# dronefreak/CABiNet

Hardware: AMD Instinct MI355X
Metric: 1024x1024 images/sec fwd+bwd (CABiNet-MobileNetV3-Large) (higher is better)
Workload: dtype f32; 1 GPU; BASELINE configs[2]: CABiNet-MobileNetV3-Large, 8x3x1024x1024 synthetic 8-class per GPU, fwd + 2x OhemCE + bwd + grad all-reduce + SGD step, HIP CAB/FFM kernels, fp32, random-init (model seed 0, gamma=0.5); per_gpu_batch=8, global_batch=8, n_classes=8, parallelism=dp1, miopen_find_mode=FAST

## Files before the change

### cabinet_amd/csrc/pwconv.hip

```cpp
#include "common.hpp"

namespace cabinet {

constexpr int PW_MAXB = 4;

template <int MB>
__global__ __launch_bounds__(64) void pw_stream_kernel(const float* __restrict__ a, int sm, int sk, int M, int K,
                                                        const float* __restrict__ x, int P, int nblocks,
                                                        int blocks_per_img, float* __restrict__ y) {
    extern __shared__ __attribute__((aligned(16))) float al[];
    const int lane = threadIdx.x, li = lane & 31, h = lane >> 5, ld = K + 1;
    for (int i0 = 0; i0 < 32 * MB * K; i0 += 64 * 8) {
        float v[8];
#pragma unroll
        for (int j = 0; j < 8; ++j) {
            const int i = i0 + j * 64 + lane, m = i / K, k = i - m * K;
            v[j] = (i < 32 * MB * K && m < M) ? a[(size_t)m * sm + (size_t)k * sk] : 0.f;
        }
#pragma unroll
        for (int j = 0; j < 8; ++j) {
            const int i = i0 + j * 64 + lane, m = i / K, k = i - m * K;
            if (i < 32 * MB * K) al[m * ld + k] = v[j];
        }
    }
    __syncthreads();
    for (int blk = blockIdx.x; blk < nblocks; blk += gridDim.x) {
        const int b = blk / blocks_per_img, p0 = (blk - b * blocks_per_img) * 64;
        const float* xb = x + (size_t)b * K * P;
        const int pa = min(p0 + li, P - 1), pb = min(p0 + 32 + li, P - 1);
        f32x16 acc[MB][2];
#pragma unroll
        for (int i = 0; i < MB; ++i)
#pragma unroll
            for (int j = 0; j < 2; ++j)
#pragma unroll
                for (int r = 0; r < 16; ++r) acc[i][j][r] = 0.f;
        for (int k0 = 0; k0 < K; k0 += 8) {
            float b0[4], b1[4];
#pragma unroll
            for (int s = 0; s < 4; ++s) {
                const float* row = xb + (size_t)(k0 + 2 * s + h) * P;
                b0[s] = row[pa];
                b1[s] = row[pb];
            }
#pragma unroll
            for (int s = 0; s < 4; ++s) {
#pragma unroll
                for (int i = 0; i < MB; ++i) {
                    const float av = al[(32 * i + li) * ld + k0 + 2 * s + h];
                    acc[i][0] = mfma32(av, b0[s], acc[i][0]);
                    acc[i][1] = mfma32(av, b1[s], acc[i][1]);
                }
            }
        }
        float* yb = y + (size_t)b * M * P;
#pragma unroll
        for (int i = 0; i < MB; ++i)
#pragma unroll
            for (int r = 0; r < 16; ++r) {
                const int m = 32 * i + acc_row(r) + 4 * h;
                if (m < M) {
                    if (p0 + li < P) yb[(size_t)m * P + p0 + li] = acc[i][0][r];
                    if (p0 + 32 + li < P) yb[(size_t)m * P + p0 + 32 + li] = acc[i][1][r];
                }
            }
    }
}

template <int COB, int CIB>
__global__ __launch_bounds__(64) void pw_wgrad_kernel(const float* __restrict__ dy, const float* __restrict__ x, int Co,
                                                       int Ci, int P, int nchunks, int chunks_per_img,
                                                       float* __restrict__ slabs) {
    extern __shared__ __attribute__((aligned(16))) float tl[];
    float* ty = tl;
    float* tx = tl + 32 * COB * 65;
    const int lane = threadIdx.x, li = lane & 31, h = lane >> 5;
    for (int i = lane; i < (32 * COB + 32 * CIB) * 65; i += 64) tl[i] = 0.f;
    f32x16 acc[COB][CIB];
#pragma unroll
    for (int i = 0; i < COB; ++i)
#pragma unroll
        for (int j = 0; j < CIB; ++j)
#pragma unroll
            for (int r = 0; r < 16; ++r) acc[i][j][r] = 0.f;
    for (int ch = blockIdx.x; ch < nchunks; ch += gridDim.x) {
        const int b = ch / chunks_per_img, p0 = (ch - b * chunks_per_img) * 64;
        const bool live = p0 + lane < P;
        const float* dyb = dy + (size_t)b * Co * P + p0 + lane;
        const float* xb = x + (size_t)b * Ci * P + p0 + lane;
        __syncthreads();
        auto stage = [&](const float* src, float* dst, int rows) {
            for (int r0 = 0; r0 < rows; r0 += 16) {
                float v[16];
#pragma unroll
                for (int j = 0; j < 16; ++j) v[j] = (live && r0 + j < rows) ? src[(size_t)(r0 + j) * P] : 0.f;
#pragma unroll
                for (int j = 0; j < 16; ++j)
                    if (r0 + j < rows) dst[(r0 + j) * 65 + lane] = v[j];
            }
        };
        stage(dyb, ty, Co);
        stage(xb, tx, Ci);
        __syncthreads();
#pragma unroll 4
        for (int s = 0; s < 32; ++s) {
            float av[COB], bv[CIB];
#pragma unroll
            for (int i = 0; i < COB; ++i) av[i] = ty[(32 * i + li) * 65 + 2 * s + h];
#pragma unroll
            for (int j = 0; j < CIB; ++j) bv[j] = tx[(32 * j + li) * 65 + 2 * s + h];
#pragma unroll
            for (int i = 0; i < COB; ++i)
#pragma unroll
                for (int j = 0; j < CIB; ++j) acc[i][j] = mfma32(av[i], bv[j], acc[i][j]);
        }
    }
    float* slab = slabs + (size_t)blockIdx.x * Co * Ci;
#pragma unroll
    for (int i = 0; i < COB; ++i)
#pragma unroll
        for (int j = 0; j < CIB; ++j)
#pragma unroll
            for (int r = 0; r < 16; ++r) {
                const int co = 32 * i + acc_row(r) + 4 * h, ci = 32 * j + li;
                if (co < Co && ci < Ci) slab[(size_t)co * Ci + ci] = acc[i][j][r];
            }
}

__global__ __launch_bounds__(256) void pw_slab_sum_kernel(const float* __restrict__ slabs, int nslab, int count,
                                                           float* __restrict__ dw) {
    const int i = blockIdx.x * 4 + (threadIdx.x >> 6), lane = threadIdx.x & 63;
    if (i >= count) return;
    float s0 = 0.f, s1 = 0.f;
    int k = lane;
    for (; k + 64 < nslab; k += 128) {
        s0 += slabs[(size_t)k * count + i];
        s1 += slabs[(size_t)(k + 64) * count + i];
    }
    if (k < nslab) s0 += slabs[(size_t)k * count + i];
    const float t = wave_sum(s0 + s1);
    if (lane == 0) dw[i] = t;
}

static int blocks_of(int n) { return ceil_div(n, 32); }
constexpr int PW_GRID = 256 * 8;

bool pwconv_supported(int Ci, int Co, int P) {
    (void)P;
    return Ci % 8 == 0 && Co % 8 == 0 && Ci <= 32 * PW_MAXB && Co <= 32 * PW_MAXB &&
           blocks_of(Ci) * blocks_of(Co) <= 8 && 32 * PW_MAXB * (Ci > Co ? Ci + 1 : Co + 1) * 4 <= 64 * 1024;
}

static int wgrad_slabs(int B, int P) {
    const int nchunks = B * ceil_div(P, 64);
    return nchunks < PW_GRID ? nchunks : PW_GRID;
}
size_t pwconv_bwd_workspace(int B, int Ci, int Co, int P) {
    return align_up((size_t)wgrad_slabs(B, P) * Co * Ci * sizeof(float), 256);
}

static hipError_t stream_launch(const float* a, int sm, int sk, int M, int K, const float* x, int B, int P, float* y,
                                hipStream_t stream) {
    const int bpi = ceil_div(P, 64), nblocks = B * bpi, grid = nblocks < PW_GRID ? nblocks : PW_GRID;
    const int mb = blocks_of(M);
    const size_t lds = (size_t)32 * mb * (K + 1) * sizeof(float);
#define PW_STREAM(MBV)                                                                                               \
    hipLaunchKernelGGL(pw_stream_kernel<MBV>, dim3(grid), dim3(64), lds, stream, a, sm, sk, M, K, x, P, nblocks, bpi, y)
    if (mb == 1) PW_STREAM(1);
    else if (mb == 2) PW_STREAM(2);
    else if (mb == 3) PW_STREAM(3);
    else PW_STREAM(4);
#undef PW_STREAM
    return hipGetLastError();
}

hipError_t pwconv_fwd_run(const float* x, const float* w, int B, int Ci, int Co, int P, float* y, hipStream_t stream) {
    return stream_launch(w, Ci, 1, Co, Ci, x, B, P, y, stream);
}

template <int COB>
static void wgrad_launch_ci(int cib, int grid, size_t lds, hipStream_t stream, const float* dy, const float* x, int Co,
                            int Ci, int P, int nchunks, int cpi, float* slabs) {
#define PW_WG(CIBV)                                                                                                    \
    hipLaunchKernelGGL((pw_wgrad_kernel<COB, CIBV>), dim3(grid), dim3(64), lds, stream, dy, x, Co, Ci, P, nchunks, cpi, \
                       slabs)
    if (cib == 1) PW_WG(1);
    else if (cib == 2) PW_WG(2);
    else if (cib == 3) { if constexpr (COB <= 2) PW_WG(3); }
    else { if constexpr (COB <= 2) PW_WG(4); }
#undef PW_WG
}

hipError_t pwconv_bwd_run(const float* dy, const float* x, const float* w, int B, int Ci, int Co, int P, float* dx,
                          float* dw, void* ws, hipStream_t stream) {
    if (dx) {
        hipError_t e = stream_launch(w, 1, Ci, Ci, Co, dy, B, P, dx, stream);
        if (e != hipSuccess) return e;
    }
    if (dw) {
        const int cpi = ceil_div(P, 64), nchunks = B * cpi, grid = wgrad_slabs(B, P);
        const int cob = blocks_of(Co), cib = blocks_of(Ci);
        const size_t lds = (size_t)(32 * cob + 32 * cib) * 65 * sizeof(float);
        float* slabs = static_cast<float*>(ws);
        if (cob == 1) wgrad_launch_ci<1>(cib, grid, lds, stream, dy, x, Co, Ci, P, nchunks, cpi, slabs);
        else if (cob == 2) wgrad_launch_ci<2>(cib, grid, lds, stream, dy, x, Co, Ci, P, nchunks, cpi, slabs);
        else if (cob == 3) wgrad_launch_ci<3>(cib, grid, lds, stream, dy, x, Co, Ci, P, nchunks, cpi, slabs);
        else wgrad_launch_ci<4>(cib, grid, lds, stream, dy, x, Co, Ci, P, nchunks, cpi, slabs);
        hipLaunchKernelGGL(pw_slab_sum_kernel, dim3(ceil_div(Co * Ci, 4)), dim3(256), 0, stream, slabs, grid, Co * Ci, dw);
    }
    return hipGetLastError();
}

}
```

Baseline: 364.1 images/s.

## Software-pipeline pointwise conv streaming loads and add opt-in fused backward kernel

```diff
diff --git a/cabinet_amd/csrc/pwconv.hip b/cabinet_amd/csrc/pwconv.hip
--- a/cabinet_amd/csrc/pwconv.hip
+++ b/cabinet_amd/csrc/pwconv.hip
@@ -1,4 +1,5 @@
 #include "common.hpp"
+#include "slab_sum.hpp"
 
 namespace cabinet {
 
@@ -24,47 +25,230 @@
         }
     }
     __syncthreads();
-    for (int blk = blockIdx.x; blk < nblocks; blk += gridDim.x) {
+    int lblk = blockIdx.x, lk = 0, lpa = 0, lpb = 0;
+    const float* lxb = x;
+    const int row_bytes = P * (int)sizeof(float);
+    auto set_block = [&](int blk) {
         const int b = blk / blocks_per_img, p0 = (blk - b * blocks_per_img) * 64;
-        const float* xb = x + (size_t)b * K * P;
-        const int pa = min(p0 + li, P - 1), pb = min(p0 + 32 + li, P - 1);
-        f32x16 acc[MB][2];
+        lpa = (h * P + min(p0 + li, P - 1)) * 4, lpb = (h * P + min(p0 + 32 + li, P - 1)) * 4;
+        lxb = x + (size_t)b * K * P;
+    };
+    set_block(lblk);
+    auto load = [&](float (&b0)[4], float (&b1)[4]) {
+        const buf_rsrc r = make_rsrc(lxb + (size_t)lk * P, 0xffffffffu);
+#pragma unroll
+        for (int s = 0; s < 4; ++s) {
+            b0[s] = bload(r, lpa, 2 * s * row_bytes);
+            b1[s] = bload(r, lpb, 2 * s * row_bytes);
+        }
+        lk += 8;
+        if (lk == K) {
+            lk = 0;
+            if (lblk + (int)gridDim.x < nblocks) set_block(lblk += gridDim.x);
+        }
+    };
+    int cblk = blockIdx.x, ck = 0;
+    f32x16 acc[MB][2];
+    auto compute = [&](const float (&b0)[4], const float (&b1)[4]) {
+        if (cblk >= nblocks) return;
+        if (ck == 0) {
+#pragma unroll
+            for (int i = 0; i < MB; ++i)
+#pragma unroll
+                for (int j = 0; j < 2; ++j)
+#pragma unroll
+                    for (int r = 0; r < 16; ++r) acc[i][j][r] = 0.f;
+        }
+#pragma unroll
+        for (int s = 0; s < 4; ++s) {
+#pragma unroll
+            for (int i = 0; i < MB; ++i) {
+                const float av = al[(32 * i + li) * ld + ck + 2 * s + h];
+                acc[i][0] = mfma32(av, b0[s], acc[i][0]);
+                acc[i][1] = mfma32(av, b1[s], acc[i][1]);
+            }
+        }
+        ck += 8;
+        if (ck < K) return;
+        const int b = cblk / blocks_per_img, p0 = (cblk - b * blocks_per_img) * 64;
+        float* yb = y + (size_t)b * M * P;
+        const unsigned so = 4u * h * P + p0 + li;
 #pragma unroll
         for (int i = 0; i < MB; ++i)
 #pragma unroll
-            for (int j = 0; j < 2; ++j)
-#pragma unroll
-                for (int r = 0; r < 16; ++r) acc[i][j][r] = 0.f;
-        for (int k0 = 0; k0 < K; k0 += 8) {
-            float b0[4], b1[4];
-#pragma unroll
-            for (int s = 0; s < 4; ++s) {
-                const float* row = xb + (size_t)(k0 + 2 * s + h) * P;
-                b0[s] = row[pa];
-                b1[s] = row[pb];
-            }
-#pragma unroll
-            for (int s = 0; s < 4; ++s) {
-#pragma unroll
-                for (int i = 0; i < MB; ++i) {
-                    const float av = al[(32 * i + li) * ld + k0 + 2 * s + h];
-                    acc[i][0] = mfma32(av, b0[s], acc[i][0]);
-                    acc[i][1] = mfma32(av, b1[s], acc[i][1]);
+            for (int r = 0; r < 16; ++r) {
+                if (32 * i + 8 * (r >> 2) < M) {
+                    float* row = yb + (size_t)(32 * i + acc_row(r)) * P;
+                    if (p0 + li < P) row[so] = acc[i][0][r];
+                    if (p0 + 32 + li < P) row[so + 32] = acc[i][1][r];
                 }
             }
-        }
-        float* yb = y + (size_t)b * M * P;
-#pragma unroll
-        for (int i = 0; i < MB; ++i)
+        ck = 0, cblk += gridDim.x;
+    };
+    float a0[4], a1[4], b0[4], b1[4], c0[4], c1[4];
+    load(a0, a1);
+    load(b0, b1);
+    while (cblk < nblocks) {
+        load(c0, c1);
+        compute(a0, a1);
+        load(a0, a1);
+        compute(b0, b1);
+        load(b0, b1);
+        compute(c0, c1);
+    }
+}
+
+constexpr int PW_LD = 65;
+
+template <int COB, int CIB, bool DX>
+__global__ __launch_bounds__(64) void pw_bwd_kernel(const float* __restrict__ dy, const float* __restrict__ x,
+                                                     const float* __restrict__ w, int Co, int Ci, int P, int nchunks,
+                                                     int chunks_per_img, float* __restrict__ dx, float* __restrict__ slabs) {
+    extern __shared__ __attribute__((aligned(16))) float tl[];
+    float* ty = tl;
+    float* tx = tl + Co * PW_LD;
+    float* wt = tx + Ci * PW_LD;
+    const int lane = threadIdx.x, li = lane & 31, h = lane >> 5, ldw = Co + 1;
+
+    float vy[32 * COB], vx[32 * CIB];
+    bool live = false;
+    auto load = [&](int ch) {
+        const int b = ch / chunks_per_img, p0 = (ch - b * chunks_per_img) * 64;
+        live = p0 + lane < P;
+        const int voff = min(p0 + lane, P - 1) * 4, row_bytes = P * (int)sizeof(float);
+        const buf_rsrc ry = make_rsrc(dy + (size_t)b * Co * P, 0xffffffffu);
+        const buf_rsrc rx = make_rsrc(x + (size_t)b * Ci * P, 0xffffffffu);
+#pragma unroll
+        for (int g = 0; g < 4 * COB; ++g)
+            if (8 * g < Co) {
+#pragma unroll
+                for (int j = 0; j < 8; ++j) vy[8 * g + j] = bload(ry, voff, (8 * g + j) * row_bytes);
+            }
+#pragma unroll
+        for (int g = 0; g < 4 * CIB; ++g)
+            if (8 * g < Ci) {
+#pragma unroll
+                for (int j = 0; j < 8; ++j) vx[8 * g + j] = bload(rx, voff, (8 * g + j) * row_bytes);
+            }
+    };
+    load(blockIdx.x);
+
+    if constexpr (DX) {
+        const int n = Co * Ci;
+        for (int i0 = 0; i0 < n; i0 += 64 * 8) {
+            float v[8];
+#pragma unroll
+            for (int j = 0; j < 8; ++j) {
+                const int i = i0 + j * 64 + lane;
+                v[j] = i < n ? w[i] : 0.f;
+            }
+#pragma unroll
+            for (int j = 0; j < 8; ++j) {
+                const int i = i0 + j * 64 + lane, co = i / Ci, ci = i - co * Ci;
+                if (i < n) wt[ci * ldw + co] = v[j];
+            }
+        }
+    }
+
+    int oy[COB], ox[CIB], ow[CIB];
+#pragma unroll
+    for (int i = 0; i < COB; ++i) oy[i] = min(32 * i + li, Co - 1) * PW_LD + h;
+#pragma unroll
+    for (int j = 0; j < CIB; ++j) {
+        ox[j] = min(32 * j + li, Ci - 1) * PW_LD + h;
+        ow[j] = min(32 * j + li, Ci - 1) * ldw + h;
+    }
+    f32x16 acc[COB][CIB];
+#pragma unroll
+    for (int i = 0; i < COB; ++i)
+#pragma unroll
+        for (int j = 0; j < CIB; ++j)
+#pragma unroll
+            for (int r = 0; r < 16; ++r) acc[i][j][r] = 0.f;
+
+    for (int ch = blockIdx.x; ch < nchunks; ch += gridDim.x) {
+        __syncthreads();
+#pragma unroll
+        for (int g = 0; g < 4 * COB; ++g)
+            if (8 * g < Co) {
+#pragma unroll
+                for (int j = 0; j < 8; ++j) ty[(8 * g + j) * PW_LD + lane] = live ? vy[8 * g + j] : 0.f;
+            }
+#pragma unroll
+        for (int g = 0; g < 4 * CIB; ++g)
+            if (8 * g < Ci) {
+#pragma unroll
+                for (int j = 0; j < 8; ++j) tx[(8 * g + j) * PW_LD + lane] = live ? vx[8 * g + j] : 0.f;
+            }
+        __syncthreads();
+        if (ch + (int)gridDim.x < nchunks) load(ch + gridDim.x);
+
+#pragma unroll 4
+        for (int s = 0; s < 32; ++s) {
+            float av[COB], bv[CIB];
+#pragma unroll
+            for (int i = 0; i < COB; ++i) av[i] = ty[oy[i] + 2 * s];
+#pragma unroll
+            for (int j = 0; j < CIB; ++j) bv[j] = tx[ox[j] + 2 * s];
+#pragma unroll
+            for (int i = 0; i < COB; ++i)
+#pragma unroll
+                for (int j = 0; j < CIB; ++j) acc[i][j] = mfma32(av[i], bv[j], acc[i][j]);
+        }
+
+        if constexpr (DX) {
+            constexpr int NH = CIB <= 2 ? 2 : 1;
+            const int b = ch / chunks_per_img, p0 = (ch - b * chunks_per_img) * 64;
+            float* dxb = dx + (size_t)b * Ci * P;
+#pragma unroll
+            for (int hp = 0; hp < 2; hp += NH) {
+                f32x16 dacc[CIB][NH];
+#pragma unroll
+                for (int i = 0; i < CIB; ++i)
+#pragma unroll
+                    for (int q = 0; q < NH; ++q)
+#pragma unroll
+                        for (int r = 0; r < 16; ++r) dacc[i][q][r] = 0.f;
+                for (int k0 = 0; k0 < Co; k0 += 8) {
+#pragma unroll
+                    for (int s = 0; s < 4; ++s) {
+                        const int k = k0 + 2 * s;
+                        float bq[NH];
+#pragma unroll
+                        for (int q = 0; q < NH; ++q) bq[q] = ty[(k + h) * PW_LD + 32 * (hp + q) + li];
+#pragma unroll
+                        for (int i = 0; i < CIB; ++i) {
+                            const float av = wt[ow[i] + k];
+#pragma unroll
+                            for (int q = 0; q < NH; ++q) dacc[i][q] = mfma32(av, bq[q], dacc[i][q]);
+                        }
+                    }
+                }
+                const unsigned so = 4u * h * P + p0 + 32 * hp + li;
+#pragma unroll
+                for (int i = 0; i < CIB; ++i)
+#pragma unroll
+                    for (int r = 0; r < 16; ++r) {
+                        if (32 * i + 8 * (r >> 2) < Ci) {
+                            float* row = dxb + (size_t)(32 * i + acc_row(r)) * P;
+#pragma unroll
+                            for (int q = 0; q < NH; ++q)
+                                if (p0 + 32 * (hp + q) + li < P) row[so + 32 * q] = dacc[i][q][r];
+                        }
+                    }
+            }
+        }
+    }
+    float* slab = slabs + (size_t)blockIdx.x * Co * Ci;
+#pragma unroll
+    for (int i = 0; i < COB; ++i)
+#pragma unroll
+        for (int j = 0; j < CIB; ++j)
 #pragma unroll
             for (int r = 0; r < 16; ++r) {
-                const int m = 32 * i + acc_row(r) + 4 * h;
-                if (m < M) {
-                    if (p0 + li < P) yb[(size_t)m * P + p0 + li] = acc[i][0][r];
-                    if (p0 + 32 + li < P) yb[(size_t)m * P + p0 + 32 + li] = acc[i][1][r];
-                }
-            }
-    }
+                const int co = 32 * i + acc_row(r) + 4 * h, ci = 32 * j + li;
+                if (co < Co && ci < Ci) slab[(size_t)co * Ci + ci] = acc[i][j][r];
+            }
 }
 
 template <int COB, int CIB>
@@ -127,21 +311,6 @@
             }
 }
 
-__global__ __launch_bounds__(256) void pw_slab_sum_kernel(const float* __restrict__ slabs, int nslab, int count,
-                                                           float* __restrict__ dw) {
-    const int i = blockIdx.x * 4 + (threadIdx.x >> 6), lane = threadIdx.x & 63;
-    if (i >= count) return;
-    float s0 = 0.f, s1 = 0.f;
-    int k = lane;
-    for (; k + 64 < nslab; k += 128) {
-        s0 += slabs[(size_t)k * count + i];
-        s1 += slabs[(size_t)(k + 64) * count + i];
-    }
-    if (k < nslab) s0 += slabs[(size_t)k * count + i];
-    const float t = wave_sum(s0 + s1);
-    if (lane == 0) dw[i] = t;
-}
-
 static int blocks_of(int n) { return ceil_div(n, 32); }
 constexpr int PW_GRID = 256 * 8;
 
@@ -159,8 +328,11 @@
     return align_up((size_t)wgrad_slabs(B, P) * Co * Ci * sizeof(float), 256);
 }
 
+constexpr int PW_MAX_P = 1 << 26;
+
 static hipError_t stream_launch(const float* a, int sm, int sk, int M, int K, const float* x, int B, int P, float* y,
                                 hipStream_t stream) {
+    if (P > PW_MAX_P) return hipErrorInvalidValue;
     const int bpi = ceil_div(P, 64), nblocks = B * bpi, grid = nblocks < PW_GRID ? nblocks : PW_GRID;
     const int mb = blocks_of(M);
     const size_t lds = (size_t)32 * mb * (K + 1) * sizeof(float);
@@ -191,23 +363,76 @@
 #undef PW_WG
 }
 
+struct PwBwdArgs {
+    const float *dy, *x, *w;
+    int Co, Ci, P, nchunks, cpi;
+    float *dx, *slabs;
+    int grid;
+    size_t lds;
+    hipStream_t stream;
+};
+
+template <int COB, int CIB, bool DX>
+static hipError_t bwd_launch_one(const PwBwdArgs& a) {
+    if (a.lds > 64 * 1024) {
+        static lds_attr_mask mask{0};
+        if (hipError_t e = ensure_dynamic_lds(reinterpret_cast<const void*>(pw_bwd_kernel<COB, CIB, DX>), 160 * 1024, mask);
+            e != hipSuccess)
+            return e;
+    }
+    hipLaunchKernelGGL((pw_bwd_kernel<COB, CIB, DX>), dim3(a.grid), dim3(64), a.lds, a.stream, a.dy, a.x, a.w, a.Co, a.Ci, a.P,
+                       a.nchunks, a.cpi, a.dx, a.slabs);
+    return hipSuccess;
+}
+
+template <int COB, bool DX>
+static hipError_t bwd_launch_ci(int cib, const PwBwdArgs& a) {
+    if (cib == 1) return bwd_launch_one<COB, 1, DX>(a);
+    if (cib == 2) return bwd_launch_one<COB, 2, DX>(a);
+    if constexpr (COB <= 2) {
+        if (cib == 3) return bwd_launch_one<COB, 3, DX>(a);
+        return bwd_launch_one<COB, 4, DX>(a);
+    }
+    return hipErrorInvalidValue;
+}
+
+template <bool DX>
+static hipError_t bwd_launch(int cob, int cib, const PwBwdArgs& a) {
+    if (cob == 1) return bwd_launch_ci<1, DX>(cib, a);
+    if (cob == 2) return bwd_launch_ci<2, DX>(cib, a);
+    if (cob == 3) return bwd_launch_ci<3, DX>(cib, a);
+    return bwd_launch_ci<4, DX>(cib, a);
+}
+
+static bool pw_fused_fits(int Ci, int Co, int P) { return (size_t)(Ci > Co ? Ci : Co) * P <= ((size_t)1 << 29); }
+
+static bool fused_bwd_plan() {
+    const char* e = getenv("CABINET_PWCONV_FUSED_BWD");
+    return e && e[0] == '1';
+}
+
 hipError_t pwconv_bwd_run(const float* dy, const float* x, const float* w, int B, int Ci, int Co, int P, float* dx,
                           float* dw, void* ws, hipStream_t stream) {
-    if (dx) {
-        hipError_t e = stream_launch(w, 1, Ci, Ci, Co, dy, B, P, dx, stream);
-        if (e != hipSuccess) return e;
-    }
-    if (dw) {
-        const int cpi = ceil_div(P, 64), nchunks = B * cpi, grid = wgrad_slabs(B, P);
-        const int cob = blocks_of(Co), cib = blocks_of(Ci);
+    if (!dw) return dx ? stream_launch(w, 1, Ci, Ci, Co, dy, B, P, dx, stream) : hipSuccess;
+    const int cpi = ceil_div(P, 64), nchunks = B * cpi, grid = wgrad_slabs(B, P);
+    const int cob = blocks_of(Co), cib = blocks_of(Ci);
+    float* slabs = static_cast<float*>(ws);
+    if (fused_bwd_plan() && pw_fused_fits(Ci, Co, P)) {
+        const size_t lds = ((size_t)(Co + Ci) * PW_LD + (dx ? (size_t)Ci * (Co + 1) : 0)) * sizeof(float);
+        const PwBwdArgs a{dy, x, w, Co, Ci, P, nchunks, cpi, dx, slabs, grid, lds, stream};
+        if (hipError_t e = dx ? bwd_launch<true>(cob, cib, a) : bwd_launch<false>(cob, cib, a); e != hipSuccess) return e;
+    } else {
+        if (dx) {
+            hipError_t e = stream_launch(w, 1, Ci, Ci, Co, dy, B, P, dx, stream);
+            if (e != hipSuccess) return e;
+        }
         const size_t lds = (size_t)(32 * cob + 32 * cib) * 65 * sizeof(float);
-        float* slabs = static_cast<float*>(ws);
         if (cob == 1) wgrad_launch_ci<1>(cib, grid, lds, stream, dy, x, Co, Ci, P, nchunks, cpi, slabs);
         else if (cob == 2) wgrad_launch_ci<2>(cib, grid, lds, stream, dy, x, Co, Ci, P, nchunks, cpi, slabs);
         else if (cob == 3) wgrad_launch_ci<3>(cib, grid, lds, stream, dy, x, Co, Ci, P, nchunks, cpi, slabs);
         else wgrad_launch_ci<4>(cib, grid, lds, stream, dy, x, Co, Ci, P, nchunks, cpi, slabs);
-        hipLaunchKernelGGL(pw_slab_sum_kernel, dim3(ceil_div(Co * Ci, 4)), dim3(256), 0, stream, slabs, grid, Co * Ci, dw);
-    }
+    }
+    slab_sum_launch(slabs, grid, Co * Ci, dw, stream);
     return hipGetLastError();
 }
 
```

Measured after the change: 366.2 images/s (median of 6 runs). About the same (+0.6%).
